# wkvong/multimodal-baby

Hardware: AMD Instinct MI355X
Metric: image-text pairs/sec, CVCL ResNeXt+embed 224², bs256, 1/2/4/8 MI355X (higher is better)
Workload: dtype bf16; 1 GPU; C2 = BASELINE configs[1]: CVCL saycam_contrastive, frozen random-init ResNeXt-50 32x4d (BN train mode) + embedding mean-pool text encoder, E=512, L2-normalised, fixed tau 0.07, 224x224 frames + 3-word utterances; full step = fwd + InfoNCE + bwd(fc, embedding) + AdamW; per_gpu_batch=256, global_batch=256, negatives=local (single GPU), parallelism=dp1, trunk_streams=2

## Files before the change

multimodal-baby_amd/csrc/resnext.hip:

```cpp
#include <algorithm>
#include <array>
#include <cstdlib>
#include <type_traits>

#include "cvcl_common.h"

namespace {

constexpr int kMaxStatsRows = 1024;
constexpr size_t kTrunkAccLayer = (size_t)kBnAccRows * 2 * 2048;


__global__ __launch_bounds__(1024) void bn_finalize_kernel(const float* __restrict__ stats, int rows, double count,
                                                           const float* __restrict__ gamma, const float* __restrict__ beta,
                                                           float* __restrict__ running_mean, float* __restrict__ running_var,
                                                           int64_t* __restrict__ nbt, float momentum, float eps,
                                                           float* __restrict__ scale, float* __restrict__ shift, int C,
                                                           float* __restrict__ moments, int moments_ld,
                                                           const float* __restrict__ centre) {
    constexpr int NS = 64, NC = 16;
    __shared__ double ps[NS][NC], pq[NS][NC];
    const int c = threadIdx.x & (NC - 1), sl = threadIdx.x / NC, ch = blockIdx.x * NC + c;
    double s = 0.0, q = 0.0;
    if (ch < C) {
// ... 415 lines not shown
            *reinterpret_cast<u16x8*>(y + (((long)b * Hp + p0 + pr) * Wp + pc) * 64 + c8 * 8) = m;
        }
    }
}

__global__ __launch_bounds__(256) void stem_direct_f32_kernel(const float* __restrict__ x, const float* __restrict__ w,
                                                              float* __restrict__ y, const float* __restrict__ centre,
                                                              int B, int Hin, int Win) {
    const int Ho = Hin / 2, Wo = Win / 2;
    const long total = (long)B * Ho * Wo * 64;
    for (long i = (long)blockIdx.x * blockDim.x + threadIdx.x; i < total; i += (long)gridDim.x * blockDim.x) {
        const int co = (int)(i & 63);
        const long p = i >> 6;
        const int ox = (int)(p % Wo), oy = (int)((p / Wo) % Ho), b = (int)(p / ((long)Wo * Ho));
        float acc = centre ? -centre[co] : 0.f;
        for (int c = 0; c < 3; ++c)
            for (int ky = 0; ky < 7; ++ky) {
                const int yin = 2 * oy - 3 + ky;
                if (yin < 0 || yin >= Hin) continue;
                for (int kx = 0; kx < 7; ++kx) {
                    const int xin = 2 * ox - 3 + kx;
                    if (xin < 0 || xin >= Win) continue;
                    acc = fmaf(x[(((long)b * 3 + c) * Hin + yin) * Win + xin], w[((co * 3 + c) * 7 + ky) * 7 + kx], acc);
                }
            }
        y[i] = acc;
    }
}

__global__ __launch_bounds__(256) void stem_tiled_f32_kernel(const float* __restrict__ x, const float* __restrict__ w,
                                                             float* __restrict__ y, const float* __restrict__ centre,
                                                             int B, int Hin, int Win, int TH, int bands) {
    extern __shared__ __attribute__((aligned(16))) float smf[];
    const int Ho = Hin / 2, Wo = Win / 2;
    const int Wp = Win + 6, rows_in = 2 * TH + 5, plane = rows_in * Wp;
    float* ws = smf;
    float* cs = ws + 147 * 64;
    float* xs = cs + 64;
    const int tid = threadIdx.x, lane = tid & 63;
    const int wave = __builtin_amdgcn_readfirstlane(tid >> 6);
    for (int e = tid; e < 147 * 64; e += 256) {
        const int co = e / 147, tap = e - co * 147;
        ws[tap * 64 + co] = w[e];
    }
    if (tid < 64) cs[tid] = centre ? -centre[tid] : 0.f;
    for (int item = blockIdx.x; item < B * bands; item += gridDim.x) {
        const int b = item / bands, band = item - b * bands;
        const int oy0 = band * TH, iy0 = 2 * oy0 - 3;
        __syncthreads();
        for (int e = tid; e < 3 * plane; e += 256) {
            const int c = e / plane, r = e - c * plane, ry = r / Wp, rx = r - ry * Wp;
            const int yin = iy0 + ry, xin = rx - 3;
            float v = 0.f;
            if ((unsigned)yin < (unsigned)Hin && (unsigned)xin < (unsigned)Win) v = x[(((long)b * 3 + c) * Hin + yin) * Win + xin];
            xs[e] = v;
        }
        __syncthreads();
        const int n_out = min(TH, Ho - oy0) * Wo, nblk = (n_out + 63) / 64;
        for (int u = wave; u < 4 * nblk; u += 4) {
            const int chunk = u / nblk, blk = u - chunk * nblk;
            const int q = blk * 64 + lane;
            const bool ok = q < n_out;
            const int qq = ok ? q : 0, ty = qq / Wo, ox = qq - ty * Wo;
            float acc[16];
#pragma unroll
            for (int o = 0; o < 16; ++o) acc[o] = cs[chunk * 16 + o];
            const float* xb = xs + (2 * ty) * Wp + 2 * ox;
            const float* wb = ws + chunk * 16;
            for (int c = 0; c < 3; ++c)
                for (int ky = 0; ky < 7; ++ky) {
#pragma unroll
                    for (int kx = 0; kx < 7; ++kx) {
                        const float xv = xb[c * plane + ky * Wp + kx];
                        const float* wt = wb + ((c * 7 + ky) * 7 + kx) * 64;
#pragma unroll
                        for (int o4 = 0; o4 < 4; ++o4) {
                            const f32x4 w4 = *reinterpret_cast<const f32x4*>(wt + o4 * 4);
#pragma unroll
                            for (int k = 0; k < 4; ++k) acc[o4 * 4 + k] = fmaf(xv, w4[k], acc[o4 * 4 + k]);
                        }
                    }
                }
            if (ok) {
                float* dst = y + (((long)b * Ho + oy0 + ty) * Wo + ox) * 64 + chunk * 16;
#pragma unroll
                for (int o4 = 0; o4 < 4; ++o4)
                    *reinterpret_cast<f32x4*>(dst + o4 * 4) = f32x4{acc[o4 * 4], acc[o4 * 4 + 1], acc[o4 * 4 + 2], acc[o4 * 4 + 3]};
            }
        }
    }
}

constexpr int POOL_ROWS = 2;
template <typename T>
__global__ __launch_bounds__(256) void bn_relu_maxpool_kernel(const T* __restrict__ x, const float* __restrict__ scale,
                                                              const float* __restrict__ shift, T* __restrict__ y,
                                                              int B, int H, int W, int C) {
    constexpr int R = POOL_ROWS, NR = 2 * R + 1, NTAP = 3 * NR;
    const int Ho = (H + 2 - 3) / 2 + 1, Wo = (W + 2 - 3) / 2 + 1, CC = C / 8;
    const int Hq = (Ho + R - 1) / R;
    const long total = (long)B * Hq * Wo * CC;
    for (long i = (long)blockIdx.x * blockDim.x + threadIdx.x; i < total; i += (long)gridDim.x * blockDim.x) {
        const int cc = (int)(i % CC);
        const long p = i / CC;
        const int ox = (int)(p % Wo), oq = (int)((p / Wo) % Hq), b = (int)(p / ((long)Wo * Hq));
        const int oy = R * oq;
        float sc[8], sh[8], m[R][8];
#pragma unroll
        for (int e = 0; e < 8; ++e) {
            sc[e] = scale[cc * 8 + e]; sh[e] = shift[cc * 8 + e];
#pragma unroll
            for (int r = 0; r < R; ++r) m[r][e] = 0.f;
        }
        constexpr int EPC = ElemTraits<T>::kPerChunk, NC = 8 / EPC;
        Chunk<T> tap[NTAP][NC];
        const T* src[NTAP];
#pragma unroll
        for (int ky = 0; ky < NR; ++ky)
#pragma unroll
            for (int kx = 0; kx < 3; ++kx) {
                const int yin = min(max(2 * oy - 1 + ky, 0), H - 1);
                const int xin = min(max(2 * ox - 1 + kx, 0), W - 1);
                src[ky * 3 + kx] = x + (((long)b * H + yin) * W + xin) * C + cc * 8;
            }
        __builtin_amdgcn_sched_barrier(0);
#pragma unroll
        for (int t = 0; t < NTAP; ++t)
#pragma unroll
            for (int q = 0; q < NC; ++q) tap[t][q].load(src[t] + q * EPC);
        __builtin_amdgcn_sched_barrier(0);
#pragma unroll
        for (int t = 0; t < NTAP; ++t)
#pragma unroll
            for (int e = 0; e < 8; ++e) {
                const float v = fmaf(tap[t][e / EPC].get(e % EPC), sc[e], sh[e]);
#pragma unroll
                for (int r = 0; r < R; ++r)
                    if (t >= 6 * r && t < 6 * r + 9) m[r][e] = fmaxf(m[r][e], v);
            }
#pragma unroll
        for (int r = 0; r < R; ++r) {
            if (oy + r < Ho) {
                T* dst = y + (((long)b * Ho + oy + r) * Wo + ox) * C + cc * 8;
#pragma unroll
                for (int e = 0; e < 8; ++e) dst[e] = ElemTraits<T>::from_f(m[r][e]);
            }
        }
    }
}

constexpr int GC_CS = 64;
constexpr int GC_PIXB = 144;

struct GconvDev {
    const void* x; const float* a_scale; const float* a_shift; const void* w; void* y; float* stats;
    const float* centre;
    int B, H, W, C, cg, stride, Ho, Wo, TH, bands, rows_in;
    float act_floor;
    BnSrc src;
    int stats_acc;
};

template <bool WIDE, int NPF, int NMT>
__global__ __launch_bounds__(256, WIDE ? 2 : 3) void gconv_mfma_kernel(GconvDev p) {
    extern __shared__ __attribute__((aligned(16))) char smem[];
    const bf16_t* __restrict__ x = (const bf16_t*)p.x;
    bf16_t* __restrict__ y = (bf16_t*)p.y;
    const int tid = threadIdx.x, lane = tid & 63, wave = tid >> 6;
    const int pix = lane & 15, kb = lane >> 4;
    const int slab = blockIdx.y, c0 = slab * GC_CS;
    const int Wp = p.W + 2;
    constexpr bool wide = WIDE;
    constexpr int KS = WIDE ? 9 : 5;
    const int unit = c0 / 16 + wave;
    const bf16_t* wu = (const bf16_t*)p.w + (long)unit * KS * 512;
    bf16x8 wf[KS];
#pragma unroll
    for (int ks = 0; ks < KS; ++ks) wf[ks] = *reinterpret_cast<const bf16x8*>(wu + (ks * 16 + pix) * 32 + kb * 8);
    const int in_ch_off = wide ? ((wave >> 1) * 32 + kb * 8) : (wave * 16 + (kb & 1) * 8);

    const int s_chunk = tid & 7, s_pix0 = tid >> 3;
    f32x2 sc[4], sh[4];
    if (p.src.acc) {
        float* aff = reinterpret_cast<float*>(smem);
        bn_slice_affine<GC_CS>(p.src, c0, blockIdx.x == 0, aff, aff + 64);
#pragma unroll
        for (int e = 0; e < 4; ++e) {
            const int cl = s_chunk * 8 + 2 * e;
            sc[e] = f32x2{aff[cl], aff[cl + 1]};
            sh[e] = f32x2{aff[64 + cl], aff[64 + cl + 1]};
        }
        __syncthreads();
    } else {
#pragma unroll
        for (int e = 0; e < 4; ++e) {
            const int ch = c0 + s_chunk * 8 + 2 * e;
            sc[e] = p.a_scale ? f32x2{p.a_scale[ch], p.a_scale[ch + 1]} : f32x2{1.f, 1.f};
            sh[e] = p.a_scale ? f32x2{p.a_shift[ch], p.a_shift[ch + 1]} : f32x2{0.f, 0.f};
        }
    }
    const bool relu_in = p.act_floor == 0.f;
    f32x2 ssum[2] = {f32x2{0.f, 0.f}, f32x2{0.f, 0.f}}, ssq[2] = {f32x2{0.f, 0.f}, f32x2{0.f, 0.f}};

    const int npix_in = p.rows_in * Wp;
    const int n_out = p.TH * p.Wo, n_mt = cvcl_div_up(n_out, 16);
    int tap_off[KS];
#pragma unroll
    for (int ks = 0; ks < KS; ++ks) {
        int tap = wide ? ks : 2 * ks + (kb >> 1);
        if (tap > 8) tap = 8;
        const int ky = tap / 3, kx = tap - ky * 3;
        tap_off[ks] = (ky * Wp + kx) * GC_PIXB + in_ch_off * 2;
    }
    int mtab[NMT];
#pragma unroll
    for (int mt = 0; mt < NMT; ++mt) {
        const int q = pix + 16 * mt;
        const bool ok = mt < n_mt && q < n_out;
        const int ty = q / p.Wo, ox = q - ty * p.Wo;
        mtab[mt] = ok ? ((((ty * p.stride) * Wp + ox * p.stride) * GC_PIXB) | (ty << 16) | (1 << 24)) : 0;
    }
    char* s_out = smem + npix_in * GC_PIXB;
    u32x4 pf[NPF];
    bool pf_in[NPF];
    int slot_y[NPF], slot_xoff[NPF];
    bool slot_ok[NPF];
#pragma unroll
    for (int i = 0; i < NPF; ++i) {
        const int pi = s_pix0 + 32 * i;
        const int pc = min(pi, npix_in - 1);
        const int ry = pc / Wp, xin = pc - ry * Wp - 1;
        slot_y[i] = ry;
        slot_ok[i] = pi < npix_in && xin >= 0 && xin < p.W;
        slot_xoff[i] = min(max(xin, 0), p.W - 1) * p.C;
    }
    const int row_elems = p.W * p.C;
    auto prefetch = [&](int item) {
        const int b = item / p.bands, band = item - b * p.bands;
        const int iy0 = band * p.TH * p.stride - 1;
        const bf16_t* xb = x + (long)b * p.H * p.W * p.C + c0 + s_chunk * 8;
#pragma unroll
        for (int i = 0; i < NPF; ++i) {
            const int yin = iy0 + slot_y[i];
            pf_in[i] = slot_ok[i] && (unsigned)yin < (unsigned)p.H;
            const int yc = min(max(yin, 0), p.H - 1);
            pf[i] = *reinterpret_cast<const u32x4*>(xb + (yc * row_elems + slot_xoff[i]));
        }
    };
    f32x4 acc_init = {0.f, 0.f, 0.f, 0.f};
    if (p.centre) {
        const f32x4 cv = *reinterpret_cast<const f32x4*>(p.centre + c0 + wave * 16 + kb * 4);
        acc_init = f32x4{-cv[0], -cv[1], -cv[2], -cv[3]};
    }
    const int n_items = p.B * p.bands;
    const int st_off = (tid >> 3) * p.C + (tid & 7) * 8;
    __builtin_amdgcn_s_waitcnt(0x0F70);
    const int bx = (gridDim.x & 7) == 0 ? (int)((blockIdx.x & 7) * (gridDim.x >> 3) + (blockIdx.x >> 3)) : (int)blockIdx.x;
    if (bx < n_items) prefetch(bx);
    for (int item = bx; item < n_items; item += gridDim.x) {
        const int b = item / p.bands, band = item - b * p.bands;
        const int oy0 = band * p.TH;
        __syncthreads();
        auto stage = [&](auto RELU) __attribute__((always_inline)) {
#pragma unroll
            for (int i = 0; i < NPF; ++i) {
                const int pi = s_pix0 + 32 * i;
                const unsigned keep = pf_in[i] ? 0xffffffffu : 0u;
                u32x4 v;
#pragma unroll
                for (int e = 0; e < 4; ++e) {
                    unsigned y = round2(__builtin_elementwise_fma(widen2(pf[i][e]), sc[e], sh[e]));
                    if constexpr (decltype(RELU)::value) y = relu2(y);
                    v[e] = y & keep;
                }
                if (pi < npix_in) *reinterpret_cast<u32x4*>(smem + pi * GC_PIXB + s_chunk * 16) = v;
            }
        };
        if (relu_in) stage(std::true_type{});
        else stage(std::false_type{});
        __syncthreads();
        if (item + (int)gridDim.x < n_items) prefetch(item + gridDim.x);
        const int rows_left = p.Ho - oy0;
#pragma unroll
        for (int mt = 0; mt < NMT; mt += 2) {
            if (mt >= n_mt) break;
            const int e0 = mtab[mt], e1 = mtab[mt + 1];
            const int base0 = e0 & 0xffff, base1 = e1 & 0xffff;
            const int q0 = pix + 16 * mt, q1 = q0 + 16;
            const bool wr0 = (e0 >> 24) && ((e0 >> 16) & 0xff) < rows_left, wr1 = (e1 >> 24) && ((e1 >> 16) & 0xff) < rows_left;
            f32x4 acc0 = acc_init, acc1 = acc_init;
#pragma unroll
            for (int ks = 0; ks < KS; ++ks) {
                const bf16x8 a0 = *reinterpret_cast<const bf16x8*>(smem + base0 + tap_off[ks]);
                const bf16x8 a1 = *reinterpret_cast<const bf16x8*>(smem + base1 + tap_off[ks]);
                acc0 = __builtin_amdgcn_mfma_f32_16x16x32_bf16(wf[ks], a0, acc0, 0, 0, 0);
                acc1 = __builtin_amdgcn_mfma_f32_16x16x32_bf16(wf[ks], a1, acc1, 0, 0, 0);
            }
            if (wr0) {
                const u32x2 o = {round2(f32x2{acc0[0], acc0[1]}), round2(f32x2{acc0[2], acc0[3]})};
                *reinterpret_cast<u32x2*>(s_out + q0 * GC_PIXB + wave * 32 + kb * 8) = o;
#pragma unroll
                for (int e = 0; e < 2; ++e) { const f32x2 sv = widen2(o[e]); ssum[e] += sv; ssq[e] = __builtin_elementwise_fma(sv, sv, ssq[e]); }
            }
            if (wr1) {
                const u32x2 o = {round2(f32x2{acc1[0], acc1[1]}), round2(f32x2{acc1[2], acc1[3]})};
                *reinterpret_cast<u32x2*>(s_out + q1 * GC_PIXB + wave * 32 + kb * 8) = o;
#pragma unroll
                for (int e = 0; e < 2; ++e) { const f32x2 sv = widen2(o[e]); ssum[e] += sv; ssq[e] = __builtin_elementwise_fma(sv, sv, ssq[e]); }
            }
        }
        __syncthreads();
        const int valid_rows = min(p.TH, p.Ho - oy0);
        const int n_chunks = valid_rows * p.Wo * 8;
        bf16_t* yb = y + ((long)b * p.Ho + oy0) * p.Wo * p.C + c0 + st_off;
        const char* so = s_out + (tid >> 3) * GC_PIXB + (tid & 7) * 16;
#pragma unroll
        for (int k = 0; k < NMT / 2; ++k) {
            if (tid + 256 * k < n_chunks)
                *reinterpret_cast<bf16x8*>(yb + (long)k * 32 * p.C) = *reinterpret_cast<const bf16x8*>(so + k * 32 * GC_PIXB);
        }
    }
#pragma unroll
    for (int e = 0; e < 4; ++e) {
        float s = ssum[e >> 1][e & 1], q = ssq[e >> 1][e & 1];
#pragma unroll
        for (int o = 1; o < 16; o <<= 1) { s += __shfl_xor(s, o, 64); q += __shfl_xor(q, o, 64); }
        if (pix == 0 && p.stats) {
            const int ch = c0 + wave * 16 + kb * 4 + e;
            cvcl_bn_stats_out(p.stats, p.stats_acc, blockIdx.x, p.C, ch, s, q);
        }
    }
}

__global__ __launch_bounds__(256) void gconv_direct_f32_kernel(const float* __restrict__ x, const float* __restrict__ a_scale,
                                                               const float* __restrict__ a_shift, const float* __restrict__ w,
                                                               float* __restrict__ y, const float* __restrict__ centre,
                                                               int B, int H, int W, int C, int cg,
                                                               int stride, int Ho, int Wo, float act_floor) {
    const long total = (long)B * Ho * Wo * C;
    for (long i = (long)blockIdx.x * blockDim.x + threadIdx.x; i < total; i += (long)gridDim.x * blockDim.x) {
        const int co = (int)(i % C);
        const long pp = i / C;
        const int ox = (int)(pp % Wo), oy = (int)((pp / Wo) % Ho), b = (int)(pp / ((long)Wo * Ho));
        const int g0 = (co / cg) * cg;
        float acc = centre ? -centre[co] : 0.f;
        for (int ci = 0; ci < cg; ++ci) {
            const float sc = a_scale ? a_scale[g0 + ci] : 1.f, sh = a_scale ? a_shift[g0 + ci] : 0.f;
            for (int ky = 0; ky < 3; ++ky) {
                const int yin = oy * stride - 1 + ky;
                if (yin < 0 || yin >= H) continue;
                for (int kx = 0; kx < 3; ++kx) {
                    const int xin = ox * stride - 1 + kx;
                    if (xin < 0 || xin >= W) continue;
                    const float v = fmaxf(fmaf(x[(((long)b * H + yin) * W + xin) * C + g0 + ci], sc, sh), act_floor);
                    acc = fmaf(v, w[((long)co * cg + ci) * 9 + ky * 3 + kx], acc);
                }
            }
        }
        y[i] = acc;
    }
}

template <int CG>
__global__ __launch_bounds__(256) void gconv_tiled_f32_kernel(const float* __restrict__ x, const float* __restrict__ a_scale,
                                                              const float* __restrict__ a_shift, const float* __restrict__ w,
                                                              float* __restrict__ y, const float* __restrict__ centre,
                                                              int B, int H, int W, int C, int stride, int Ho, int Wo, int TH,
                                                              int bands, int plane_p, float act_floor) {
    extern __shared__ __attribute__((aligned(16))) float smf[];
    constexpr int NG = 64 / CG;
    const int Wp = W + 2, rows_in = (TH - 1) * stride + 3, plane = rows_in * Wp;
    float* ws = smf;
    float* cs = ws + 64 * 9 * CG;
    float* xs = cs + 64;
    const int c0 = blockIdx.y * 64;
    const int tid = threadIdx.x, lane = tid & 63;
    const int wave = __builtin_amdgcn_readfirstlane(tid >> 6);
    for (int e = tid; e < 64 * CG * 9; e += 256) {
        const int co = e / (CG * 9), r = e - co * (CG * 9), ci = r / 9, tap = r - ci * 9;
        const int g = co / CG, o = co - g * CG;
        ws[((g * 9 + tap) * CG + ci) * CG + o] = w[(long)c0 * CG * 9 + e];
    }
    if (tid < 64) cs[tid] = centre ? -centre[c0 + tid] : 0.f;
    const int ch4 = tid & 15;
    f32x4 sc4 = {1.f, 1.f, 1.f, 1.f}, sh4 = {0.f, 0.f, 0.f, 0.f};
    if (a_scale) {
        sc4 = *reinterpret_cast<const f32x4*>(a_scale + c0 + ch4 * 4);
        sh4 = *reinterpret_cast<const f32x4*>(a_shift + c0 + ch4 * 4);
    }
    for (int item = blockIdx.x; item < B * bands; item += gridDim.x) {
        const int b = item / bands, band = item - b * bands;
        const int oy0 = band * TH, iy0 = oy0 * stride - 1;
        __syncthreads();
        for (int pix = tid >> 4; pix < plane; pix += 16) {
            const int ry = pix / Wp, rx = pix - ry * Wp;
            const int yin = iy0 + ry, xin = rx - 1;
            f32x4 v = {0.f, 0.f, 0.f, 0.f};
            if ((unsigned)yin < (unsigned)H && (unsigned)xin < (unsigned)W) {
                v = *reinterpret_cast<const f32x4*>(x + (((long)b * H + yin) * W + xin) * C + c0 + ch4 * 4);
                if (a_scale) {
#pragma unroll
                    for (int k = 0; k < 4; ++k) v[k] = fmaxf(fmaf(v[k], sc4[k], sh4[k]), act_floor);
                }
            }
#pragma unroll
            for (int k = 0; k < 4; ++k) xs[(ch4 * 4 + k) * plane_p + pix] = v[k];
        }
        __syncthreads();
        const int n_out = min(TH, Ho - oy0) * Wo, nblk = (n_out + 63) / 64;
        for (int u = wave; u < NG * nblk; u += 4) {
            const int g = u / nblk, blk = u - g * nblk;
            const int q = blk * 64 + lane;
            const bool ok = q < n_out;
            const int qq = ok ? q : 0, ty = qq / Wo, ox = qq - ty * Wo;
            float acc[CG];
#pragma unroll
            for (int o = 0; o < CG; ++o) acc[o] = cs[g * CG + o];
            const float* xb = xs + (g * CG) * plane_p + (ty * stride) * Wp + ox * stride;
            const float* wb = ws + g * 9 * CG * CG;
#pragma unroll
            for (int tap = 0; tap < 9; ++tap) {
                const int ky = tap / 3, kx = tap - ky * 3;
#pragma unroll 4
                for (int ci = 0; ci < CG; ++ci) {
                    const float xv = xb[ci * plane_p + ky * Wp + kx];
                    const float* wt = wb + (tap * CG + ci) * CG;
#pragma unroll
                    for (int o4 = 0; o4 < CG / 4; ++o4) {
                        const f32x4 w4 = *reinterpret_cast<const f32x4*>(wt + o4 * 4);
#pragma unroll
                        for (int k = 0; k < 4; ++k) acc[o4 * 4 + k] = fmaf(xv, w4[k], acc[o4 * 4 + k]);
                    }
                }
            }
            if (ok) {
                float* dst = y + (((long)b * Ho + oy0 + ty) * Wo + ox) * C + c0 + g * CG;
#pragma unroll
                for (int o4 = 0; o4 < CG / 4; ++o4)
                    *reinterpret_cast<f32x4*>(dst + o4 * 4) = f32x4{acc[o4 * 4], acc[o4 * 4 + 1], acc[o4 * 4 + 2], acc[o4 * 4 + 3]};
            }
        }
    }
}

template <typename T>
__global__ __launch_bounds__(256) void bn_add_relu_kernel(const T* __restrict__ raw, const float* __restrict__ scale,
                                                          const float* __restrict__ shift, const T* __restrict__ idn,
                                                          const float* __restrict__ idn_scale,
                                                          const float* __restrict__ idn_shift, T* __restrict__ out,
                                                          long rows, int C) {
    constexpr int EPC = ElemTraits<T>::kPerChunk;
    const int CC = C / EPC;
    const long total = rows * CC;
    const long i0 = (long)blockIdx.x * blockDim.x + threadIdx.x;
    const int c = (int)(i0 % CC) * EPC;
    float sc[EPC], sh[EPC], isc[EPC], ish[EPC];
    const float* isp = idn_scale ? idn_scale : scale;
    const float* ihp = idn_scale ? idn_shift : shift;
#pragma unroll
// ... 277 lines not shown
    return 0;
}

extern "C" int cvcl_pack_conv_weight(int dtype, int kind, const float* w_oihw, void* out, int cout, int cin_per_group,
                                     int k, void* stream) {
    CVCL_CHECK_DTYPE_TRUNK(dtype, "cvcl_pack_conv_weight");
    CVCL_CHECK_ARG(w_oihw && out && cout > 0 && cin_per_group > 0, "cvcl_pack_conv_weight: bad args");
    CvclProfScope prof(stream, CVCL_K_OTHER);
    hipStream_t s = (hipStream_t)stream;
    const long n = (long)cout * cin_per_group * k * k;
    if (dtype == CVCL_F32X3) {
        if (kind == CVCL_PACK_DENSE) return cvcl_pack_split_dense(w_oihw, out, n, stream);
        if (kind == CVCL_PACK_STEM7) {
            CVCL_CHECK_ARG(cout == 64 && cin_per_group == 3 && k == 7, "cvcl_pack_conv_weight: stem must be 64x3x7x7");
            return cvcl_pack_split_conv(1, w_oihw, out, cout, 3, stream);
        }
        if (kind == CVCL_PACK_GCONV3) {
            CVCL_CHECK_ARG(k == 3, "cvcl_pack_conv_weight: grouped conv must be 3x3");
            return cvcl_pack_split_conv(0, w_oihw, out, cout, cin_per_group, stream);
        }
        cvcl_set_error("cvcl_pack_conv_weight: unknown kind %d", kind);
        return CVCL_EINVAL;
    }
    if (dtype == CVCL_F32) {
        hipLaunchKernelGGL(cast_kernel<float>, dim3(cvcl_grid(n, 256, 4096)), dim3(256), 0, s, w_oihw, (float*)out, n);
    } else if (kind == CVCL_PACK_DENSE) {
        hipLaunchKernelGGL(cast_kernel<bf16_t>, dim3(cvcl_grid(n, 256, 4096)), dim3(256), 0, s, w_oihw, (bf16_t*)out, n);
    } else if (kind == CVCL_PACK_STEM7) {
        CVCL_CHECK_ARG(cout == 64 && cin_per_group == 3 && k == 7, "cvcl_pack_conv_weight: stem must be 64x3x7x7");
        hipLaunchKernelGGL(pack_stem_kernel, dim3(cvcl_div_up(4 * 6 * 512, 256)), dim3(256), 0, s, w_oihw, (bf16_t*)out);
    } else if (kind == CVCL_PACK_GCONV3) {
        CVCL_CHECK_ARG(k == 3 && (cin_per_group == 4 || cin_per_group == 8 || cin_per_group == 16 || cin_per_group == 32) &&
                           cout % 64 == 0, "cvcl_pack_conv_weight: unsupported grouped conv %d/%d", cout, cin_per_group);
        const long total = (long)(cout / 16) * (cin_per_group == 32 ? 9 : 5) * 512;
        hipLaunchKernelGGL(pack_gconv_kernel, dim3(cvcl_div_up(total, 256)), dim3(256), 0, s, w_oihw, (bf16_t*)out, cout,
                           cin_per_group);
    } else {
        cvcl_set_error("cvcl_pack_conv_weight: unknown kind %d", kind);
        return CVCL_EINVAL;
    }
    CVCL_LAUNCH_CHECK();
    return CVCL_OK;
}

static int stem_grid(int B, int Hin) {
    const int items = B * cvcl_div_up(Hin / 2, STEM_TH);
    return items < 512 ? items : 512;
}

extern "C" int cvcl_stem_conv_stats_rows(int dtype, int B, int H, int W) {
    if (!cvcl_dtype_trunk(dtype)) return 0;
    if (dtype == CVCL_F32X3) return cvcl_stem_split_stats_rows(B, H, W);
    if (dtype == CVCL_BF16) return stem_grid(B, H);
    return cvcl_col_stats_rows((long)B * (H / 2) * (W / 2));
}

extern "C" int cvcl_stem_conv7x7(int dtype, const float* x_nchw, const void* w_packed, void* y_nhwc, float* stats,
                                 int stats_rows, const float* centre, int B, int H, int W, void* stream) {
    CVCL_CHECK_DTYPE_TRUNK(dtype, "cvcl_stem_conv7x7");
    if (dtype == CVCL_F32X3)
        return cvcl_stem_split(x_nchw, w_packed, (float*)y_nhwc, stats, stats_rows, centre, B, H, W, stream);
    CVCL_CHECK_ARG(x_nchw && w_packed && (y_nhwc || (dtype == CVCL_BF16 && stats)) && B > 0 && H % 2 == 0 && W % 2 == 0,
                   "cvcl_stem_conv7x7: bad args");
    hipStream_t s = (hipStream_t)stream;
    if (dtype == CVCL_BF16) {
        CVCL_CHECK_ARG(W + 6 + 8 <= 2 * STEM_PITCH && W % 4 == 0 && W / 4 <= 64,
                       "cvcl_stem_conv7x7: width %d not supported by the staged patch", W);
        const int g = stem_grid(B, H);
        CVCL_CHECK_ARG(!stats || stats_rows >= g, "cvcl_stem_conv7x7: stats_rows %d < %d", stats_rows, g);
        const size_t lds = (size_t)3 * STEM_ROWS * STEM_PITCH * 4 + 4 * 16 * STEM_OPITCH + 64 * 4;
        float* st = stats;
        CVCL_CHECK_ARG(st, "cvcl_stem_conv7x7: the bf16 kernel always emits statistics; pass a buffer");
        CvclProfScope prof(stream, CVCL_K_STEM);
        hipLaunchKernelGGL(stem_mfma_kernel, dim3(g), dim3(256), lds, s, x_nchw, (const bf16_t*)w_packed, (bf16_t*)y_nhwc,
                           st, centre, B, H, W);
        CVCL_LAUNCH_CHECK();
        return CVCL_OK;
    }
    const long total = (long)B * (H / 2) * (W / 2) * 64;
    {
        CvclProfScope prof(stream, CVCL_K_STEM);
        const int Ho = H / 2;
        auto lds_of = [&](int th) { return (size_t)(147 * 64 + 64 + 3 * (2 * th + 5) * (W + 6)) * 4; };
        int TH = Ho < 8 ? Ho : 8;
        while (TH > 1 && lds_of(TH) > 150 * 1024) --TH;
        if (lds_of(TH) <= 150 * 1024) {
            static CvclLdsAttr attr;
            if (const int rc = cvcl_raise_lds_limit(attr, (const void*)stem_tiled_f32_kernel, 160 * 1024, "cvcl_stem_conv7x7")) return rc;
            attr.mark();
            const int bands = cvcl_div_up(Ho, TH);
            const long items = (long)B * bands;
            hipLaunchKernelGGL(stem_tiled_f32_kernel, dim3((unsigned)(items < 1024 ? items : 1024)), dim3(256), lds_of(TH), s, x_nchw,
                               (const float*)w_packed, (float*)y_nhwc, centre, B, H, W, TH, bands);
        } else {
            hipLaunchKernelGGL(stem_direct_f32_kernel, dim3(cvcl_grid(total, 256, 8192)), dim3(256), 0, s, x_nchw,
                               (const float*)w_packed, (float*)y_nhwc, centre, B, H, W);
        }
    }
    CVCL_LAUNCH_CHECK();
    if (stats) return cvcl_col_stats(CVCL_F32, y_nhwc, (long)B * (H / 2) * (W / 2), 64, stats, stats_rows, stream);
    return CVCL_OK;
}

extern "C" int cvcl_stem_pool_supported(int dtype, int H, int W) {
    return dtype == CVCL_BF16 && H % 2 == 0 && W % 4 == 0 && W / 4 <= 64 && W + 6 + 8 <= 2 * STEM_PITCH && W / 2 + 2 <= STEMP_BW;
}

extern "C" int cvcl_stem_pool(int dtype, const float* x_nchw, const void* w_packed, const float* scale, const float* shift,
                              const float* centre, void* y_nhwc, int B, int H, int W, void* stream) {
    CVCL_CHECK_DTYPE(dtype, "cvcl_stem_pool");
    CVCL_CHECK_ARG(x_nchw && w_packed && scale && shift && y_nhwc && B > 0, "cvcl_stem_pool: bad args");
    CVCL_CHECK_ARG(cvcl_stem_pool_supported(dtype, H, W), "cvcl_stem_pool: bf16 and a width <= %d only (got dtype %d, %d x %d)",
                   2 * (STEMP_BW - 2), dtype, H, W);
    const size_t lds = (size_t)3 * STEMP_ROWS * STEM_PITCH * 4 + (size_t)STEMP_CR * STEMP_BW * 128 + 3 * 64 * 4;
    static CvclLdsAttr attr;
    if (const int rc = cvcl_raise_lds_limit(attr, (const void*)stem_pool_mfma_kernel, (int)lds, "cvcl_stem_pool")) return rc;
    attr.mark();
    const int Hp = (H / 2 - 1) / 2 + 1;
    const int items = B * cvcl_div_up(Hp, STEMP_TP);
    int dev = 0, cus = 256;
    if (hipGetDevice(&dev) != hipSuccess || hipDeviceGetAttribute(&cus, hipDeviceAttributeMultiprocessorCount, dev) != hipSuccess || cus <= 0) cus = 256;
    const int grid = items < cus ? items : cus;
    CvclProfScope prof(stream, CVCL_K_STEM);
    hipLaunchKernelGGL(stem_pool_mfma_kernel, dim3(grid), dim3(512), lds, (hipStream_t)stream, x_nchw, (const bf16_t*)w_packed,
                       (bf16_t*)y_nhwc, scale, shift, centre, B, H, W);
    CVCL_LAUNCH_CHECK();
    return CVCL_OK;
}

extern "C" int cvcl_bn_relu_maxpool(int dtype, const void* x, const float* scale, const float* shift, void* y, int B,
                                    int H, int W, int C, void* stream) {
    CVCL_CHECK_DTYPE_TRUNK(dtype, "cvcl_bn_relu_maxpool");
    dtype = cvcl_storage_dtype(dtype);
    CVCL_CHECK_ARG(x && scale && shift && y && C % 8 == 0, "cvcl_bn_relu_maxpool: bad args");
    CvclProfScope prof(stream, CVCL_K_MAXPOOL);
    const int Ho = (H - 1) / 2 + 1, Wo = (W - 1) / 2 + 1;
    const long total = (long)B * ((Ho + POOL_ROWS - 1) / POOL_ROWS) * Wo * (C / 8);
    const int grid = cvcl_grid(total, 256, 8192);
    if (dtype == CVCL_F32)
        hipLaunchKernelGGL(bn_relu_maxpool_kernel<float>, dim3(grid), dim3(256), 0, (hipStream_t)stream,
                           (const float*)x, scale, shift, (float*)y, B, H, W, C);
    else
        hipLaunchKernelGGL(bn_relu_maxpool_kernel<bf16_t>, dim3(grid), dim3(256), 0, (hipStream_t)stream,
                           (const bf16_t*)x, scale, shift, (bf16_t*)y, B, H, W, C);
    CVCL_LAUNCH_CHECK();
    return CVCL_OK;
}

namespace {
struct GconvPlan { int TH, bands, rows_in, grid_x; size_t lds; };
GconvPlan gconv_plan(int B, int H, int W, int C, int stride) {
    GconvPlan g;
    const int Ho = (H - 1) / stride + 1, Wo = (W - 1) / stride + 1, Wp = W + 2;
    auto bytes = [&](int th) { return (size_t)(((th - 1) * stride + 3) * Wp + th * Wo) * GC_PIXB; };
    int TH = Ho;
    while (TH > 1 && (bytes(TH) > (size_t)52 * 1024 || ((TH - 1) * stride + 3) * Wp > 10 * 32 || TH * Wo > 128)) TH = (TH + 1) / 2;
    g.TH = TH;
    g.bands = cvcl_div_up(Ho, TH);
    g.rows_in = (TH - 1) * stride + 3;
    g.lds = bytes(TH);
    int per_cu = (int)((160 * 1024) / g.lds);
    const int reg_limit = (C / 32 == 32) ? 2 : 3;
    if (per_cu > reg_limit) per_cu = reg_limit;
    if (per_cu < 1) per_cu = 1;
    const int slabs = C / GC_CS;
    int gx = per_cu * 256 / slabs;
    if (gx < 1) gx = 1;
    const int items = B * g.bands;
    g.grid_x = items < gx ? items : gx;
    return g;
}
}

extern "C" int cvcl_gconv3x3_stats_rows(int dtype, int B, int H, int W, int C, int stride) {
    if (!cvcl_dtype_trunk(dtype)) return 0;
    if (dtype == CVCL_F32X3) return C % 32 == 0 ? cvcl_gconv_split_stats_rows(B, H, W, C, stride) : 0;
    if (dtype == CVCL_BF16) return gconv_plan(B, H, W, C, stride).grid_x;
    const int Ho = (H - 1) / stride + 1, Wo = (W - 1) / stride + 1;
    return cvcl_col_stats_rows((long)B * Ho * Wo);
}

static int gconv3x3_impl(int dtype, const void* x, const float* a_scale, const float* a_shift, const BnSrc* src, const void* w_packed,
                         void* y, float* stats, int stats_rows, const float* centre, int B, int H, int W, int C, int groups,
                         int stride, void* stream) {
    CVCL_CHECK_DTYPE_TRUNK(dtype, "cvcl_gconv3x3");
    CVCL_CHECK_ARG(x && w_packed && y && (!a_scale == !a_shift), "cvcl_gconv3x3: null pointer");
    CVCL_CHECK_ARG(!src || (dtype == CVCL_BF16 && src->acc && src->gamma && src->beta && src->C == C && src->count > 0 &&
                            (const void*)src->acc != (const void*)stats),
                   "cvcl_gconv3x3: finalize-on-load source");
    CVCL_CHECK_ARG(stats_rows != CVCL_STATS_ACCUMULATE || dtype == CVCL_BF16, "cvcl_gconv3x3: accumulators exist for bf16 only");
    const float act_floor = (a_scale || src) ? 0.f : -INFINITY;
    CVCL_CHECK_ARG(B > 0 && (stride == 1 || stride == 2) && groups > 0 && C % groups == 0, "cvcl_gconv3x3: bad shape");
    const int cg = C / groups;
    const int Ho = (H - 1) / stride + 1, Wo = (W - 1) / stride + 1;
    hipStream_t s = (hipStream_t)stream;
    if (dtype == CVCL_F32X3)
        return cvcl_gconv_split((const float*)x, a_scale, a_shift, act_floor, w_packed, (float*)y, stats, stats_rows, centre, B, H, W, C,
                                cg, stride, stream);
    if (dtype == CVCL_BF16) {
        CVCL_CHECK_ARG((cg == 4 || cg == 8 || cg == 16 || cg == 32) && C % GC_CS == 0,
                       "cvcl_gconv3x3: unsupported channels-per-group %d (C=%d)", cg, C);
        const GconvPlan g = gconv_plan(B, H, W, C, stride);
        CVCL_CHECK_ARG(g.lds <= 160 * 1024 && g.rows_in * (W + 2) <= 10 * 32 && g.TH * ((W - 1) / stride + 1) <= 128,
                       "cvcl_gconv3x3: feature map too wide for one staged band (%zu B, %d pixels)", g.lds, g.rows_in * (W + 2));
        CVCL_CHECK_ARG(!stats || stats_rows == CVCL_STATS_ACCUMULATE || stats_rows >= g.grid_x, "cvcl_gconv3x3: stats_rows %d < %d", stats_rows, g.grid_x);
        GconvDev d;
        d.x = x; d.a_scale = a_scale; d.a_shift = a_shift; d.w = w_packed; d.y = y; d.stats = stats; d.centre = centre;
        d.B = B; d.H = H; d.W = W; d.C = C; d.cg = cg; d.stride = stride; d.Ho = Ho; d.Wo = Wo;
        d.TH = g.TH; d.bands = g.bands; d.rows_in = g.rows_in;
        d.act_floor = act_floor;
        d.src = BnSrc{};
        d.stats_acc = stats && stats_rows == CVCL_STATS_ACCUMULATE;
        if (src) {
            CVCL_CHECK_ARG(g.lds >= 2048, "cvcl_gconv3x3: band buffers smaller than the finalize-on-load scratch");
            d.src = *src;
        }
        CvclProfScope prof(stream, CVCL_K_GCONV);
        int rc;
        const int slots = cvcl_div_up(g.rows_in * (W + 2), 32);
        static CvclLdsAttr attr_set[2][2][11];
        auto launch = [&](auto kern) -> int {
            CvclLdsAttr& done = attr_set[cg == 32][g.TH * Wo <= 64][slots <= 4 ? 4 : slots <= 6 ? 6 : slots <= 8 ? 8 : 10];
            if (const int rc = cvcl_raise_lds_limit(done, (const void*)kern, 160 * 1024, "cvcl_gconv3x3")) return rc;
            done.mark();
            hipLaunchKernelGGL(kern, dim3(g.grid_x, C / GC_CS), dim3(256), g.lds, s, d);
            return CVCL_OK;
        };
        const bool few = g.TH * Wo <= 64;
#define CVCL_GCONV_PICK(W_) \
        (slots <= 4 ? (few ? launch(gconv_mfma_kernel<W_, 4, 4>) : launch(gconv_mfma_kernel<W_, 4, 8>)) \
         : slots <= 6 ? (few ? launch(gconv_mfma_kernel<W_, 6, 4>) : launch(gconv_mfma_kernel<W_, 6, 8>)) \
         : slots <= 8 ? (few ? launch(gconv_mfma_kernel<W_, 8, 4>) : launch(gconv_mfma_kernel<W_, 8, 8>)) \
                      : (few ? launch(gconv_mfma_kernel<W_, 10, 4>) : launch(gconv_mfma_kernel<W_, 10, 8>)))
        rc = cg == 32 ? CVCL_GCONV_PICK(true) : CVCL_GCONV_PICK(false);
#undef CVCL_GCONV_PICK
        if (rc) return rc;
        CVCL_LAUNCH_CHECK();
        return CVCL_OK;
    }
    const long total = (long)B * Ho * Wo * C;
    {
        CvclProfScope prof(stream, CVCL_K_GCONV);
        auto plane_p_of = [&](int th) { const int pl = ((th - 1) * stride + 3) * (W + 2); return pl + ((9 - (pl & 7)) & 7); };
        auto lds_of = [&](int th) { return (size_t)(64 * 9 * cg + 64 + 64 * plane_p_of(th)) * 4; };
        int TH = Ho;
        while (TH > 1 && lds_of(TH) > 150 * 1024) --TH;
        const bool tiled = C % 64 == 0 && (cg == 4 || cg == 8 || cg == 16 || cg == 32) && lds_of(TH) <= 150 * 1024 &&
                           ((uintptr_t)x & 15) == 0 && ((uintptr_t)y & 15) == 0 && ((uintptr_t)a_scale & 15) == 0 && ((uintptr_t)a_shift & 15) == 0;
        if (tiled) {
            const int bands = cvcl_div_up(Ho, TH);
            const long items = (long)B * bands;
            const int slabs = C / 64;
            long gx = 1024 / slabs;
            if (gx < 1) gx = 1;
            if (gx > items) gx = items;
            static CvclLdsAttr attr[4];
            auto launch = [&](auto kern, int slot) -> int {
                if (const int rc = cvcl_raise_lds_limit(attr[slot], (const void*)kern, 160 * 1024, "cvcl_gconv3x3")) return rc;
                attr[slot].mark();
                hipLaunchKernelGGL(kern, dim3((unsigned)gx, slabs), dim3(256), lds_of(TH), s, (const float*)x, a_scale, a_shift,
                                   (const float*)w_packed, (float*)y, centre, B, H, W, C, stride, Ho, Wo, TH, bands, plane_p_of(TH), act_floor);
                return CVCL_OK;
            };
            const int rc = cg == 4 ? launch(gconv_tiled_f32_kernel<4>, 0) : cg == 8 ? launch(gconv_tiled_f32_kernel<8>, 1)
                         : cg == 16 ? launch(gconv_tiled_f32_kernel<16>, 2) : launch(gconv_tiled_f32_kernel<32>, 3);
            if (rc) return rc;
        } else {
            hipLaunchKernelGGL(gconv_direct_f32_kernel, dim3(cvcl_grid(total, 256, 8192)), dim3(256), 0, s, (const float*)x, a_scale,
                               a_shift, (const float*)w_packed, (float*)y, centre, B, H, W, C, cg, stride, Ho, Wo, act_floor);
        }
    }
    CVCL_LAUNCH_CHECK();
    if (stats) return cvcl_col_stats(CVCL_F32, y, (long)B * Ho * Wo, C, stats, stats_rows, stream);
    return CVCL_OK;
}

extern "C" int cvcl_gconv3x3(int dtype, const void* x, const float* a_scale, const float* a_shift, const void* w_packed,
                             void* y, float* stats, int stats_rows, const float* centre, int B, int H, int W, int C, int groups,
                             int stride, void* stream) {
    return gconv3x3_impl(dtype, x, a_scale, a_shift, nullptr, w_packed, y, stats, stats_rows, centre, B, H, W, C, groups, stride, stream);
}

extern "C" int cvcl_bn_add_relu(int dtype, const void* raw, const float* scale, const float* shift, const void* idn,
                                const float* idn_scale, const float* idn_shift, void* out, long rows, int C, void* stream) {
    CVCL_CHECK_DTYPE_TRUNK(dtype, "cvcl_bn_add_relu");
    dtype = cvcl_storage_dtype(dtype);
    CVCL_CHECK_ARG(raw && scale && shift && idn && out && rows > 0 && C % 8 == 0, "cvcl_bn_add_relu: bad args");
    CvclProfScope prof(stream, CVCL_K_BN_ADD_RELU);
    CVCL_CHECK_ARG((idn_scale == nullptr) == (idn_shift == nullptr), "cvcl_bn_add_relu: idn_scale/idn_shift pair");
    const int epc = dtype == CVCL_F32 ? 4 : 8;
    CVCL_CHECK_ARG(C % epc == 0, "cvcl_bn_add_relu: C must be a multiple of %d", epc);
    hipStream_t s = (hipStream_t)stream;
    const int cc = C / epc;
    int g256 = cc, t256 = 256;
    while (t256) { const int r = g256 % t256; g256 = t256; t256 = r; }
    const int mult = cc / g256;
    int grid = cvcl_grid(rows * (long)cc, 256 * 4, 16384);
    grid = (grid + mult - 1) / mult * mult;
    if (dtype == CVCL_F32)
        hipLaunchKernelGGL(bn_add_relu_kernel<float>, dim3(grid), dim3(256), 0, s, (const float*)raw,
                           scale, shift, (const float*)idn, idn_scale, idn_shift, (float*)out, rows, C);
    else
        hipLaunchKernelGGL(bn_add_relu_kernel<bf16_t>, dim3(grid), dim3(256), 0, s, (const bf16_t*)raw,
                           scale, shift, (const bf16_t*)idn, idn_scale, idn_shift, (bf16_t*)out, rows, C);
    CVCL_LAUNCH_CHECK();
    return CVCL_OK;
}

extern "C" int cvcl_bn_relu_apply(int dtype, const void* x, const float* scale, const float* shift, void* y, long rows,
                                  int C, void* stream) {
    CVCL_CHECK_DTYPE_TRUNK(dtype, "cvcl_bn_relu_apply");
    dtype = cvcl_storage_dtype(dtype);
    CVCL_CHECK_ARG(x && scale && shift && y && rows > 0, "cvcl_bn_relu_apply: bad args");
    CvclProfScope prof(stream, CVCL_K_BN_APPLY);
    const int epc = dtype == CVCL_F32 ? 4 : 8;
    CVCL_CHECK_ARG(C % epc == 0, "cvcl_bn_relu_apply: C must be a multiple of %d", epc);
    const int cc = C / epc;
    int g256 = cc, t256 = 256;
    while (t256) { const int r = g256 % t256; g256 = t256; t256 = r; }
    const int mult = cc / g256;
    int grid = cvcl_grid(rows * (long)cc, 256 * 4, 16384);
    grid = (grid + mult - 1) / mult * mult;
    if (dtype == CVCL_F32)
        hipLaunchKernelGGL(bn_relu_apply_kernel<float>, dim3(grid), dim3(256), 0, (hipStream_t)stream, (const float*)x, scale,
                           shift, (float*)y, rows, C);
    else
        hipLaunchKernelGGL(bn_relu_apply_kernel<bf16_t>, dim3(grid), dim3(256), 0, (hipStream_t)stream, (const bf16_t*)x,
                           scale, shift, (bf16_t*)y, rows, C);
    CVCL_LAUNCH_CHECK();
    return CVCL_OK;
}

extern "C" int cvcl_avgpool(int dtype, const void* x, float* out, int B, int HW, int C, void* stream) {
    CVCL_CHECK_DTYPE_TRUNK(dtype, "cvcl_avgpool");
    dtype = cvcl_storage_dtype(dtype);
    CVCL_CHECK_ARG(x && out && B > 0 && HW > 0 && C > 0, "cvcl_avgpool: bad args");
    CvclProfScope prof(stream, CVCL_K_AVGPOOL);
    if (dtype == CVCL_F32)
        hipLaunchKernelGGL(avgpool_kernel<float>, dim3(cvcl_grid((long)B * C, 256, 4096)), dim3(256), 0, (hipStream_t)stream, (const float*)x, out, B, HW, C);
    else
        hipLaunchKernelGGL(avgpool_kernel<bf16_t>, dim3(cvcl_grid((long)B * C, 256, 4096)), dim3(256), 0, (hipStream_t)stream, (const bf16_t*)x, out, B, HW, C);
    CVCL_LAUNCH_CHECK();
    return CVCL_OK;
}

namespace {
constexpr int kLayers[4] = {3, 4, 6, 3};
constexpr int kTrunkLayers = 53;
constexpr int kMaxC = 2048;
constexpr int kAffStride = 2 * kMaxC;
enum { kConv1, kConv2, kConv3, kDownsample };
static_assert(sizeof(EvalAffineAll::C) == sizeof(int) * kTrunkLayers && sizeof(ApplyMomentsAll::C) == sizeof(int) * kTrunkLayers,
              "the one-launch layer tables hold the whole trunk");

constexpr int block_layer_c(int stage, int j) { return (64 << stage) * (j < kConv3 ? 2 : 4); }

constexpr std::array<int, kTrunkLayers> kTrunkC = [] {
    std::array<int, kTrunkLayers> c = {64};
    int l = 1;
    for (int st = 0; st < 4; ++st)
        for (int b = 0; b < kLayers[st]; ++b)
            for (int j = 0; j < (b == 0 ? 4 : 3); ++j) c[l++] = block_layer_c(st, j);
    return c;
}();

template <class T>
T trunk_table(const cvcl_convbn_params* layers) {
    T t;
    for (int l = 0; l < kTrunkLayers; ++l) {
        const cvcl_convbn_params& p = layers[l];
        t.rm[l] = p.running_mean; t.rv[l] = p.running_var; t.C[l] = kTrunkC[l];
        if constexpr (std::is_same_v<T, EvalAffineAll>) { t.gamma[l] = p.gamma; t.beta[l] = p.beta; }
        else t.nbt[l] = p.num_batches_tracked;
    }
    return t;
}

inline size_t al256(size_t x) { return (x + 255) & ~(size_t)255; }
struct Regions {
    uintptr_t base;
    size_t end = 0;
    template <class T> T* take(size_t bytes) { T* p = (T*)(base + end); end += al256(bytes); return p; }
};
constexpr size_t kStatsBytes = (size_t)kMaxStatsRows * 2 * kMaxC * 4;
constexpr size_t kAccBytes = kTrunkAccLayer * 8;
inline size_t act_elems(int B, int H, int W) {
    return (size_t)B * (H / 2) * (W / 2) * 64;
// ... 432 lines not shown
```

Measured before the change: 51480 pairs/s.

## Add row-reuse grouped conv path sharing LDS loads via DPP lane shifts

Adds a row-reuse variant of the narrow grouped 3x3 MFMA kernel for stride-1 layers. Output tiles are 14 pixels along a row, and each K-step operand set is built from three LDS loads per tile (top, middle and bottom rows), with the column-shifted taps produced by DPP row shifts instead of separate LDS reads. The goal is to cut LDS read traffic in the inner MFMA loop. In exchange it adds DPP instructions, wastes 2 of 16 MFMA rows per tile, and changes band-height planning for stride-1 layers.

```diff
diff --git a/multimodal-baby_amd/csrc/resnext.hip b/multimodal-baby_amd/csrc/resnext.hip
--- a/multimodal-baby_amd/csrc/resnext.hip
+++ b/multimodal-baby_amd/csrc/resnext.hip
@@ -591,6 +591,29 @@
 constexpr int GC_CS = 64;
 constexpr int GC_PIXB = 144;
 
+template <int ROW_MASK>
+__device__ __forceinline__ bf16x8 gconv_rr_shl2(bf16x8 old, bf16x8 src) {
+    const u32x4 o = __builtin_bit_cast(u32x4, old), v = __builtin_bit_cast(u32x4, src);
+    u32x4 r;
+#pragma unroll
+    for (int e = 0; e < 4; ++e) r[e] = (unsigned)__builtin_amdgcn_update_dpp((int)o[e], (int)v[e], 0x102, ROW_MASK, 0xF, false);
+    return __builtin_bit_cast(bf16x8, r);
+}
+__device__ __forceinline__ void gconv_rr_operands(const char* smem, int tile, int row_b, int off_e, int off_m, bf16x8 (&a)[5]) {
+    const bf16x8 e0 = *reinterpret_cast<const bf16x8*>(smem + (tile + off_e));
+    const bf16x8 m = *reinterpret_cast<const bf16x8*>(smem + ((tile + row_b) + off_m));
+    const bf16x8 e2 = *reinterpret_cast<const bf16x8*>(smem + ((tile + 2 * row_b) + off_e));
+    a[0] = e0;
+    a[1] = gconv_rr_shl2<0x3>(m, e0);
+    a[2] = gconv_rr_shl2<0xC>(m, m);
+    a[3] = e2;
+    const u32x4 v = __builtin_bit_cast(u32x4, e2);
+    u32x4 r;
+#pragma unroll
+    for (int e = 0; e < 4; ++e) r[e] = (unsigned)__builtin_amdgcn_update_dpp(0, (int)v[e], 0x102, 0xF, 0xF, true);
+    a[4] = __builtin_bit_cast(bf16x8, r);
+}
+
 struct GconvDev {
     const void* x; const float* a_scale; const float* a_shift; const void* w; void* y; float* stats;
     const float* centre;
@@ -600,8 +623,11 @@
     int stats_acc;
 };
 
-template <bool WIDE, int NPF, int NMT>
+constexpr int GC_RR_PIX = 14;
+
+template <bool WIDE, int NPF, int NMT, bool RR = false>
 __global__ __launch_bounds__(256, WIDE ? 2 : 3) void gconv_mfma_kernel(GconvDev p) {
+    static_assert(!(WIDE && RR), "row reuse is for the two-taps-per-K-step (narrow) form");
     extern __shared__ __attribute__((aligned(16))) char smem[];
     const bf16_t* __restrict__ x = (const bf16_t*)p.x;
     bf16_t* __restrict__ y = (bf16_t*)p.y;
@@ -642,7 +668,9 @@
     f32x2 ssum[2] = {f32x2{0.f, 0.f}, f32x2{0.f, 0.f}}, ssq[2] = {f32x2{0.f, 0.f}, f32x2{0.f, 0.f}};
 
     const int npix_in = p.rows_in * Wp;
-    const int n_out = p.TH * p.Wo, n_mt = cvcl_div_up(n_out, 16);
+    const int n_out = p.TH * p.Wo;
+    const int rr_tpr = cvcl_div_up(p.Wo, GC_RR_PIX);
+    const int n_mt = RR ? p.TH * rr_tpr : cvcl_div_up(n_out, 16);
     int tap_off[KS];
 #pragma unroll
     for (int ks = 0; ks < KS; ++ks) {
@@ -651,13 +679,17 @@
         const int ky = tap / 3, kx = tap - ky * 3;
         tap_off[ks] = (ky * Wp + kx) * GC_PIXB + in_ch_off * 2;
     }
-    int mtab[NMT];
-#pragma unroll
-    for (int mt = 0; mt < NMT; ++mt) {
-        const int q = pix + 16 * mt;
-        const bool ok = mt < n_mt && q < n_out;
-        const int ty = q / p.Wo, ox = q - ty * p.Wo;
-        mtab[mt] = ok ? ((((ty * p.stride) * Wp + ox * p.stride) * GC_PIXB) | (ty << 16) | (1 << 24)) : 0;
+    const int rr_off_e = (pix + (kb >> 1)) * GC_PIXB + in_ch_off * 2, rr_off_m = (pix + 1 - (kb >> 1)) * GC_PIXB + in_ch_off * 2;
+    const int rr_out = pix * GC_PIXB + wave * 32 + kb * 8;
+    int mtab[RR ? 1 : NMT];
+    if constexpr (!RR) {
+#pragma unroll
+        for (int mt = 0; mt < NMT; ++mt) {
+            const int q = pix + 16 * mt;
+            const bool ok = mt < n_mt && q < n_out;
+            const int ty = q / p.Wo, ox = q - ty * p.Wo;
+            mtab[mt] = ok ? ((((ty * p.stride) * Wp + ox * p.stride) * GC_PIXB) | (ty << 16) | (1 << 24)) : 0;
+        }
     }
     char* s_out = smem + npix_in * GC_PIXB;
     u32x4 pf[NPF];
@@ -720,30 +752,61 @@
         __syncthreads();
         if (item + (int)gridDim.x < n_items) prefetch(item + gridDim.x);
         const int rows_left = p.Ho - oy0;
+        int rr_ty = 0, rr_j = 0;
+        if constexpr (RR) asm volatile("" : "+s"(rr_ty), "+s"(rr_j));
 #pragma unroll
         for (int mt = 0; mt < NMT; mt += 2) {
             if (mt >= n_mt) break;
-            const int e0 = mtab[mt], e1 = mtab[mt + 1];
-            const int base0 = e0 & 0xffff, base1 = e1 & 0xffff;
-            const int q0 = pix + 16 * mt, q1 = q0 + 16;
-            const bool wr0 = (e0 >> 24) && ((e0 >> 16) & 0xff) < rows_left, wr1 = (e1 >> 24) && ((e1 >> 16) & 0xff) < rows_left;
+            int base0, base1, q0, q1;
+            bool wr0, wr1;
+            if constexpr (RR) {
+                const int ty0 = rr_ty, j0 = rr_j;
+                if (++rr_j == rr_tpr) { rr_j = 0; ++rr_ty; }
+                const int ty1 = rr_ty, j1 = rr_j;
+                if (++rr_j == rr_tpr) { rr_j = 0; ++rr_ty; }
+                base0 = (ty0 * Wp + j0 * GC_RR_PIX) * GC_PIXB;
+                base1 = mt + 1 < n_mt ? (ty1 * Wp + j1 * GC_RR_PIX) * GC_PIXB : base0;
+                q0 = ty0 * p.Wo + j0 * GC_RR_PIX;
+                q1 = ty1 * p.Wo + j1 * GC_RR_PIX;
+                wr0 = ty0 < rows_left && pix < min(GC_RR_PIX, p.Wo - j0 * GC_RR_PIX);
+                wr1 = mt + 1 < n_mt && ty1 < rows_left && pix < min(GC_RR_PIX, p.Wo - j1 * GC_RR_PIX);
+            } else {
+                const int e0 = mtab[mt], e1 = mtab[mt + 1];
+                base0 = e0 & 0xffff; base1 = e1 & 0xffff;
+                q0 = pix + 16 * mt; q1 = q0 + 16;
+                wr0 = (e0 >> 24) && ((e0 >> 16) & 0xff) < rows_left;
+                wr1 = (e1 >> 24) && ((e1 >> 16) & 0xff) < rows_left;
+            }
+            char* const o0 = RR ? s_out + (q0 * GC_PIXB + rr_out) : s_out + q0 * GC_PIXB + wave * 32 + kb * 8;
+            char* const o1 = RR ? s_out + (q1 * GC_PIXB + rr_out) : s_out + q1 * GC_PIXB + wave * 32 + kb * 8;
             f32x4 acc0 = acc_init, acc1 = acc_init;
-#pragma unroll
-            for (int ks = 0; ks < KS; ++ks) {
-                const bf16x8 a0 = *reinterpret_cast<const bf16x8*>(smem + base0 + tap_off[ks]);
-                const bf16x8 a1 = *reinterpret_cast<const bf16x8*>(smem + base1 + tap_off[ks]);
-                acc0 = __builtin_amdgcn_mfma_f32_16x16x32_bf16(wf[ks], a0, acc0, 0, 0, 0);
-                acc1 = __builtin_amdgcn_mfma_f32_16x16x32_bf16(wf[ks], a1, acc1, 0, 0, 0);
+            if constexpr (RR) {
+                bf16x8 a0[KS], a1[KS];
+                gconv_rr_operands(smem, base0, Wp * GC_PIXB, rr_off_e, rr_off_m, a0);
+                gconv_rr_operands(smem, base1, Wp * GC_PIXB, rr_off_e, rr_off_m, a1);
+#pragma unroll
+                for (int ks = 0; ks < KS; ++ks) {
+                    acc0 = __builtin_amdgcn_mfma_f32_16x16x32_bf16(wf[ks], a0[ks], acc0, 0, 0, 0);
+                    acc1 = __builtin_amdgcn_mfma_f32_16x16x32_bf16(wf[ks], a1[ks], acc1, 0, 0, 0);
+                }
+            } else {
+#pragma unroll
+                for (int ks = 0; ks < KS; ++ks) {
+                    const bf16x8 a0 = *reinterpret_cast<const bf16x8*>(smem + base0 + tap_off[ks]);
+                    const bf16x8 a1 = *reinterpret_cast<const bf16x8*>(smem + base1 + tap_off[ks]);
+                    acc0 = __builtin_amdgcn_mfma_f32_16x16x32_bf16(wf[ks], a0, acc0, 0, 0, 0);
+                    acc1 = __builtin_amdgcn_mfma_f32_16x16x32_bf16(wf[ks], a1, acc1, 0, 0, 0);
+                }
             }
             if (wr0) {
                 const u32x2 o = {round2(f32x2{acc0[0], acc0[1]}), round2(f32x2{acc0[2], acc0[3]})};
-                *reinterpret_cast<u32x2*>(s_out + q0 * GC_PIXB + wave * 32 + kb * 8) = o;
+                *reinterpret_cast<u32x2*>(o0) = o;
 #pragma unroll
                 for (int e = 0; e < 2; ++e) { const f32x2 sv = widen2(o[e]); ssum[e] += sv; ssq[e] = __builtin_elementwise_fma(sv, sv, ssq[e]); }
             }
             if (wr1) {
                 const u32x2 o = {round2(f32x2{acc1[0], acc1[1]}), round2(f32x2{acc1[2], acc1[3]})};
-                *reinterpret_cast<u32x2*>(s_out + q1 * GC_PIXB + wave * 32 + kb * 8) = o;
+                *reinterpret_cast<u32x2*>(o1) = o;
 #pragma unroll
                 for (int e = 0; e < 2; ++e) { const f32x2 sv = widen2(o[e]); ssum[e] += sv; ssq[e] = __builtin_elementwise_fma(sv, sv, ssq[e]); }
             }
@@ -1327,9 +1390,12 @@
 GconvPlan gconv_plan(int B, int H, int W, int C, int stride) {
     GconvPlan g;
     const int Ho = (H - 1) / stride + 1, Wo = (W - 1) / stride + 1, Wp = W + 2;
-    auto bytes = [&](int th) { return (size_t)(((th - 1) * stride + 3) * Wp + th * Wo) * GC_PIXB; };
+    const int rr_tiles_per_row = cvcl_div_up(Wo, GC_RR_PIX);
+    auto bytes = [&](int th) { return (size_t)(((th - 1) * stride + 3) * Wp + (th * Wo > 16 ? th * Wo : 16)) * GC_PIXB; };
     int TH = Ho;
-    while (TH > 1 && (bytes(TH) > (size_t)52 * 1024 || ((TH - 1) * stride + 3) * Wp > 10 * 32 || TH * Wo > 128)) TH = (TH + 1) / 2;
+    while (TH > 1 && (bytes(TH) > (size_t)52 * 1024 || ((TH - 1) * stride + 3) * Wp > 10 * 32 || TH * Wo > 128 ||
+                      (stride == 1 && TH * rr_tiles_per_row > 8)))
+        TH = (TH + 1) / 2;
     g.TH = TH;
     g.bands = cvcl_div_up(Ho, TH);
     g.rows_in = (TH - 1) * stride + 3;
@@ -1393,21 +1459,23 @@
         CvclProfScope prof(stream, CVCL_K_GCONV);
         int rc;
         const int slots = cvcl_div_up(g.rows_in * (W + 2), 32);
-        static CvclLdsAttr attr_set[2][2][11];
+        const int rr_tiles = g.TH * cvcl_div_up(Wo, GC_RR_PIX);
+        const bool rr = stride == 1 && cg != 32 && rr_tiles <= 8;
+        const bool few = rr ? rr_tiles <= 4 : g.TH * Wo <= 64;
+        static CvclLdsAttr attr_set[3][2][11];
         auto launch = [&](auto kern) -> int {
-            CvclLdsAttr& done = attr_set[cg == 32][g.TH * Wo <= 64][slots <= 4 ? 4 : slots <= 6 ? 6 : slots <= 8 ? 8 : 10];
+            CvclLdsAttr& done = attr_set[cg == 32 ? 0 : rr ? 2 : 1][few][slots <= 4 ? 4 : slots <= 6 ? 6 : slots <= 8 ? 8 : 10];
             if (const int rc = cvcl_raise_lds_limit(done, (const void*)kern, 160 * 1024, "cvcl_gconv3x3")) return rc;
             done.mark();
             hipLaunchKernelGGL(kern, dim3(g.grid_x, C / GC_CS), dim3(256), g.lds, s, d);
             return CVCL_OK;
         };
-        const bool few = g.TH * Wo <= 64;
-#define CVCL_GCONV_PICK(W_) \
-        (slots <= 4 ? (few ? launch(gconv_mfma_kernel<W_, 4, 4>) : launch(gconv_mfma_kernel<W_, 4, 8>)) \
-         : slots <= 6 ? (few ? launch(gconv_mfma_kernel<W_, 6, 4>) : launch(gconv_mfma_kernel<W_, 6, 8>)) \
-         : slots <= 8 ? (few ? launch(gconv_mfma_kernel<W_, 8, 4>) : launch(gconv_mfma_kernel<W_, 8, 8>)) \
-                      : (few ? launch(gconv_mfma_kernel<W_, 10, 4>) : launch(gconv_mfma_kernel<W_, 10, 8>)))
-        rc = cg == 32 ? CVCL_GCONV_PICK(true) : CVCL_GCONV_PICK(false);
+#define CVCL_GCONV_PICK(W_, RR_) \
+        (slots <= 4 ? (few ? launch(gconv_mfma_kernel<W_, 4, 4, RR_>) : launch(gconv_mfma_kernel<W_, 4, 8, RR_>)) \
+         : slots <= 6 ? (few ? launch(gconv_mfma_kernel<W_, 6, 4, RR_>) : launch(gconv_mfma_kernel<W_, 6, 8, RR_>)) \
+         : slots <= 8 ? (few ? launch(gconv_mfma_kernel<W_, 8, 4, RR_>) : launch(gconv_mfma_kernel<W_, 8, 8, RR_>)) \
+                      : (few ? launch(gconv_mfma_kernel<W_, 10, 4, RR_>) : launch(gconv_mfma_kernel<W_, 10, 8, RR_>)))
+        rc = cg == 32 ? CVCL_GCONV_PICK(true, false) : rr ? CVCL_GCONV_PICK(false, true) : CVCL_GCONV_PICK(false, false);
 #undef CVCL_GCONV_PICK
         if (rc) return rc;
         CVCL_LAUNCH_CHECK();
```

New measurement: 51390 pairs/s, median of 2. Within noise of the previous version (-0.2%).
